# Harrypotterrrr/DVD-GAN

Measured on AMD Instinct MI355X. Metric: clips/sec per G+Ds+Dt step, 48x64x64 UCF-101 synth, higher is better.
Workload: dtype bf16; 1 GPU; UCF-101-shaped 101-class 48x64x64 clips, G+Ds+Dt hinge step, ch=32, k_sample=8, batch 64/GPU (BASELINE configs[1]); global_batch=64, parallelism=dp1

## Files before the change

dvd_gan_amd/csrc/conv_common.h:

```cpp
#pragma once
#include "common.h"

namespace dvdk {

constexpr int BM = 128, BN = 128, NT = 256;
constexpr int TILEB = BM * 80;
constexpr int WG_LD = 132;

__device__ __forceinline__ u32x4 relu16_f32(u32x4 v) {
    v.x = (int32_t)v.x < 0 ? 0u : v.x; v.y = (int32_t)v.y < 0 ? 0u : v.y;
    v.z = (int32_t)v.z < 0 ? 0u : v.z; v.w = (int32_t)v.w < 0 ? 0u : v.w;
    return v;
}
__device__ __forceinline__ uint32_t relu2_bf16(uint32_t v) {
    uint32_t m = ((v >> 15) & 0x00010001u) * 0xffffu;
    return v & ~m;
}
__device__ __forceinline__ u32x4 relu16_bf16(u32x4 v) {
    v.x = relu2_bf16(v.x); v.y = relu2_bf16(v.y); v.z = relu2_bf16(v.z); v.w = relu2_bf16(v.w);
    return v;
}
template <typename T> __device__ __forceinline__ u32x4 relu16(u32x4 v);
template <> __device__ __forceinline__ u32x4 relu16<float>(u32x4 v) { return relu16_f32(v); }
template <> __device__ __forceinline__ u32x4 relu16<bf16_t>(u32x4 v) { return relu16_bf16(v); }
// ... 408 lines not shown
        },
        [&](int i) __attribute__((always_inline)) {
            const int rr = rrow(i);
            float v[8], rv[8], m8[8];
            staged(i, v); unpack8(resv[i % (D + 1)], rv); unpack8(mv[i % (D + 1)], m8);
#pragma unroll
            for (int k = 0; k < 8; ++k) v[k] = (v[k] + bias8[k]) + rv[k];
            if (p.act == DVD_ACT_RELU) {
#pragma unroll
                for (int k = 0; k < 8; ++k) v[k] = fmaxf(v[k], 0.f);
            } else if (p.act == DVD_ACT_TANH) {
#pragma unroll
                for (int k = 0; k < 8; ++k) v[k] = gate_tanh<T>(v[k]);
            } else if (p.act == DVD_ACT_SIGMOID) {
#pragma unroll
                for (int k = 0; k < 8; ++k) v[k] = gate_sigmoid<T>(v[k]);
            }
#pragma unroll
            for (int k = 0; k < 8; ++k) {
                v[k] = (has_mask && !(m8[k] > 0.f)) ? 0.f : v[k];
                v[k] = (k < nvalid) ? v[k] : 0.f;
            }
            if (p.out_f32) bst8<float>(rout, offs(rr, p.ldo, 4, col, colv), v);
            else bst8<T>(rout, offs(rr, p.ldo, esz, col, colv), v);
        });
}

template <bool UP2> struct HaloGeo {
    static constexpr int PITCH = UP2 ? 12 : 20;
    static constexpr int SWA = UP2 ? 2 : 0;
    static __device__ __forceinline__ int sw(int hy, int hx) { return ((hx >> 2) + SWA * hy) & 3; }
};

constexpr int kGroupMax = 6;
struct ConvGroup {
    int n, head, nslots;
    int order[kGroupMax];
    int wgs[kGroupMax];
    ConvK c[kGroupMax];
};
static_assert(sizeof(ConvGroup) <= 3584, "ConvGroup must fit the kernel argument segment");

void launch_gb(const ConvK& p, int variant, bool relu_in, bool up2, dim3 grid, hipStream_t st);
void launch_gbs(const ConvK& p, int S, bool big, bool relu_in, dim3 grid, hipStream_t st);
void launch_group(const ConvGroup& grp, int kind, hipStream_t st);

}
using namespace dvdk;
```

dvd_gan_amd/csrc/conv_gb.hip:

```cpp
#include "conv_common.h"

namespace {

#ifndef DVD_GB_EPI_DEEP
#define DVD_GB_EPI_DEEP 0
#endif

constexpr unsigned kRowOOB = 0x80000000u, kStepOOB = 0x40000000u, kRangeCap = 0x3fffffffu;

template <int TM, int WN, int WMV, bool UP2> struct HaloGbCfg {
    static constexpr int PITCH = HaloGeo<UP2>::PITCH;
    static constexpr int NWAVE = WMV * WN;
    static constexpr int PH = WMV * TM * 2;
    static constexpr int HG = UP2 ? ((PH / 2 + 3) * PITCH + 15) / 16 : ((PH + 4) * PITCH + 15) / 16;
    static constexpr int HBYTES = HG * 1024;
    static constexpr int EPI = NWAVE * 32 * 64 * 4;
    static constexpr int LDSB = 2 * HBYTES + 1024 > EPI ? 2 * HBYTES + 1024 : EPI;
};

template <int TM, bool RELU, class LdA, class Next>
__device__ __forceinline__ void gb_step(f32x16 (&acc)[TM][2], const bf16x8 (&b)[2][2], LdA ldA, Next next) {
    constexpr int NU = 2 * TM;
#ifndef DVD_GB_ADEPTH
#define DVD_GB_ADEPTH 2
// ... 344 lines not shown
                auto next = [&]() __attribute__((always_inline)) {
                    ldBq((ix & 1) ? b0 : b1, nrec);
                    if (ix == 0 && first && more) dmaH(hb ^ 1, cc + 1);
                };
                gb_step<TM, RELU>(acc, (ix & 1) ? b1 : b0, ldA, next);
                rec = nrec;
            }
            ++iy;
            if (last) {
                iy = 0; hb ^= 1; ++cc;
                if (more) {
                    __builtin_amdgcn_s_waitcnt(0xc07f);
                    __builtin_amdgcn_s_barrier();
                }
            }
        };
        const int nrows = nch * KS;
        int r = 0;
#pragma unroll 1
        for (; r + 1 < nrows; r += 2) { row(bq0, bq1); row(bq1, bq0); }
        if (r < nrows) row(bq0, bq1);
    }
    __syncthreads();

    float* ep = reinterpret_cast<float*>(&smem[0]) + wave * (32 * 64);
    const int ecol = (lane & 7) * 8, erow = lane >> 3;
    const long long row0 = (long long)ft0 * SS;
    conv_epilogue<T, TM, DVD_GB_EPI_DEEP>(p, acc, ep, lane, n0 + wn * 64 + ecol, z, ltile, row0, [&](int tm, int j) __attribute__((always_inline)) {
        const int pi = wm * (TM * 32) + tm * 32 + j * 8 + erow;
        return row0 + pi < p.M ? pi : -1;
    });
}

template <int TM, int S, bool RELU, int KS>
__global__ __launch_bounds__(256, 2) void conv_halo_gbs_kernel(ConvK p) {
    __shared__ __attribute__((aligned(16))) char smem[HaloGbsCfg<TM, S>::LDSB];
    const int bid = xcd_order(blockIdx.x, gridDim.x);
    const TileMN t = tile_of(p.nmajor, p.tilesN, bid, gridDim.x);
    conv_halo_gbs_tile<TM, S, RELU, KS>(p, smem, t.mt, t.nt, blockIdx.z, (int)blockIdx.x);
}

template <class TileFn>
__device__ __forceinline__ void group_dispatch(const ConvGroup& grp, TileFn fn) {
    const int x = blockIdx.x & 7;
    int rem = blockIdx.x >> 3;
    auto share = [&](int m) __attribute__((always_inline)) -> int { const int w = grp.wgs[m]; return (w >> 3) + (x < (w & 7) ? 1 : 0); };
    const int m0 = grp.order[0], m1 = grp.n > 1 ? grp.order[1] : m0;
    const int s0 = share(m0), s1 = grp.n > 1 ? share(m1) : 0;
    const int h0 = min(grp.head, s0), h1 = min(grp.head, s1);
    int g = -1, off = 0;
    if (rem < h0) { g = m0; off = rem; }
    else if ((rem -= h0) < h1) { g = m1; off = rem; }
    else if ((rem -= h1) < s0 - h0) { g = m0; off = h0 + rem; }
    else if ((rem -= s0 - h0) < s1 - h1) { g = m1; off = h1 + rem; }
    else {
        rem -= s1 - h1;
        for (int k = 2; k < grp.n; ++k) {
            const int m = grp.order[k], s = share(m);
            if (rem < s) { g = m; off = rem; break; }
            rem -= s;
        }
    }
    if (g < 0) return;
    const int w = grp.wgs[g];
    const int local = x * (w >> 3) + min(x, w & 7) + off;
    const ConvK& p = grp.c[g];
    const int t = local / p.nsplit, z = local - t * p.nsplit;
    const TileMN mn = tile_of(p.nmajor, p.tilesN, t, w / p.nsplit);
    fn(p, mn.mt, mn.nt, z, t);
}

template <int TM, int WN, int WMV>
__global__ __launch_bounds__(256, 2) void conv_group_gb_kernel(ConvGroup grp) {
    __shared__ __attribute__((aligned(16))) char smem[HaloGbCfg<TM, WN, WMV, false>::LDSB];
    group_dispatch(grp, [&](const ConvK& p, int mt, int nt, int z, int t) __attribute__((always_inline)) {
        if (p.kh == 5) conv_halo_gb_tile<TM, WN, WMV, false, false, 5>(p, smem, mt, nt, z, t);
        else conv_halo_gb_tile<TM, WN, WMV, false, false, 3>(p, smem, mt, nt, z, t);
    });
}

template <int TM, int S>
__global__ __launch_bounds__(256, 2) void conv_group_gbs_kernel(ConvGroup grp) {
    __shared__ __attribute__((aligned(16))) char smem[HaloGbsCfg<TM, S>::LDSB];
    group_dispatch(grp, [&](const ConvK& p, int mt, int nt, int z, int t) __attribute__((always_inline)) {
        if (p.kh == 5) conv_halo_gbs_tile<TM, S, false, 5>(p, smem, mt, nt, z, t);
        else conv_halo_gbs_tile<TM, S, false, 3>(p, smem, mt, nt, z, t);
    });
}

struct FragK { const bf16_t* w; bf16_t* wq; int ntaps, Cout, C, kchunks, nb32; };
__global__ void fragment_major_kernel(FragK p) {
    const long long n = (long long)p.ntaps * p.kchunks * p.nb32 * 2 * 64;
    const long long i = (long long)blockIdx.x * blockDim.x + threadIdx.x;
    if (i >= n) return;
    const int l = (int)(i & 63);
    long long r = i >> 6;
    const int kk = (int)(r & 1); r >>= 1;
    const int nb = (int)(r % p.nb32); r /= p.nb32;
    const int cc = (int)(r % p.kchunks);
    const int tap = (int)(r / p.kchunks);
    const int co = nb * 32 + (l & 31), ci = cc * 32 + (kk * 2 + (l >> 5)) * 8;
    u32x4 v = {0u, 0u, 0u, 0u};
    if (co < p.Cout && ci < p.C) v = *reinterpret_cast<const u32x4*>(p.w + ((size_t)tap * p.Cout + co) * p.C + ci);
    *reinterpret_cast<u32x4*>(p.wq + i * 8) = v;
}
constexpr int kFragBatch = 32;
struct FragBatchK { FragK it[kFragBatch]; int first[kFragBatch + 1]; int n; };
__global__ void fragment_major_batched_kernel(FragBatchK b) {
    int j = 0;
    while (j + 1 < b.n && (int)blockIdx.x >= b.first[j + 1]) ++j;
    const FragK& p = b.it[j];
    const long long n = (long long)p.ntaps * p.kchunks * p.nb32 * 2 * 64;
    const long long i = (long long)((int)blockIdx.x - b.first[j]) * blockDim.x + threadIdx.x;
    if (i >= n) return;
    const int l = (int)(i & 63);
    long long r = i >> 6;
    const int kk = (int)(r & 1); r >>= 1;
// ... 1 lines not shown
    const int cc = (int)(r % p.kchunks);
    const int tap = (int)(r / p.kchunks);
    const int co = nb * 32 + (l & 31), ci = cc * 32 + (kk * 2 + (l >> 5)) * 8;
    u32x4 v = {0u, 0u, 0u, 0u};
    if (co < p.Cout && ci < p.C) v = *reinterpret_cast<const u32x4*>(p.w + ((size_t)tap * p.Cout + co) * p.C + ci);
    *reinterpret_cast<u32x4*>(p.wq + i * 8) = v;
}

}

#ifdef DVD_GB_PROBE
namespace dvdk {
void launch_gb(const ConvK& p, int, bool, bool, dim3 grid, hipStream_t st) { conv_halo_gb_kernel<4, 2, 2, false, false, 5><<<grid, 256, 0, st>>>(p); }
void launch_gbs(const ConvK& p, int, bool, bool, dim3 grid, hipStream_t st) { conv_halo_gbs_kernel<2, 8, false, 3><<<grid, 256, 0, st>>>(p); }
void launch_group(const ConvGroup& grp, int, hipStream_t st) { conv_group_gb_kernel<4, 2, 2><<<dim3(grp.nslots), 256, 0, st>>>(grp); }
}
#else
namespace dvdk {
void launch_gb(const ConvK& p, int variant, bool relu_in, bool up2, dim3 grid, hipStream_t st) {
#define LAUNCH_GB4(TM_, WN_, WMV_, KS_)                                                                       \
    do { if (relu_in) { if (up2) conv_halo_gb_kernel<TM_, WN_, WMV_, true, true, KS_><<<grid, 256, 0, st>>>(p);       \
                        else conv_halo_gb_kernel<TM_, WN_, WMV_, true, false, KS_><<<grid, 256, 0, st>>>(p); }           \
         else         { if (up2) conv_halo_gb_kernel<TM_, WN_, WMV_, false, true, KS_><<<grid, 256, 0, st>>>(p);      \
                        else conv_halo_gb_kernel<TM_, WN_, WMV_, false, false, KS_><<<grid, 256, 0, st>>>(p); } } while (0)
#define LAUNCH_GB(TM_, WN_, WMV_) do { if (p.kh == 5) LAUNCH_GB4(TM_, WN_, WMV_, 5); else LAUNCH_GB4(TM_, WN_, WMV_, 3); } while (0)
    if (variant == 2) LAUNCH_GB(2, 1, 4); else if (variant == 0) LAUNCH_GB(4, 2, 2); else LAUNCH_GB(2, 2, 2);
#undef LAUNCH_GB
#undef LAUNCH_GB4
}
void launch_gbs(const ConvK& p, int S, bool big, bool relu_in, dim3 grid, hipStream_t st) {
#define LAUNCH_GBS2(TM_, SZ_, KS_) do { if (relu_in) conv_halo_gbs_kernel<TM_, SZ_, true, KS_><<<grid, 256, 0, st>>>(p);   \
                                        else conv_halo_gbs_kernel<TM_, SZ_, false, KS_><<<grid, 256, 0, st>>>(p); } while (0)
#define LAUNCH_GBS(TM_, SZ_) do { if (p.kh == 5) LAUNCH_GBS2(TM_, SZ_, 5); else LAUNCH_GBS2(TM_, SZ_, 3); } while (0)
    if (S == 8) { if (big) LAUNCH_GBS(4, 8); else LAUNCH_GBS(2, 8); }
    else LAUNCH_GBS(2, 4);
#undef LAUNCH_GBS
#undef LAUNCH_GBS2
}
void launch_group(const ConvGroup& grp, int kind, hipStream_t st) {
    const dim3 grid(grp.nslots);
    switch (kind) {
        case 0: conv_group_gb_kernel<4, 2, 2><<<grid, 256, 0, st>>>(grp); break;
        case 1: conv_group_gb_kernel<2, 2, 2><<<grid, 256, 0, st>>>(grp); break;
        case 2: conv_group_gbs_kernel<4, 8><<<grid, 256, 0, st>>>(grp); break;
        case 3: conv_group_gbs_kernel<2, 8><<<grid, 256, 0, st>>>(grp); break;
        default: conv_group_gbs_kernel<2, 4><<<grid, 256, 0, st>>>(grp); break;
    }
}
}
#endif

extern "C" long long dvd_conv_fragment_major_bytes(int ntaps, int Cout, int C) {
    if (ntaps <= 0 || Cout <= 0 || C <= 0) return 0;
    const long long kchunks = (C + 31) / 32, nb32 = (Cout + 127) / 128 * 4;
    return (long long)ntaps * kchunks * nb32 * 2048;
}
extern "C" int dvd_conv_fragment_major(int dtype, const void* w, void* wq, int ntaps, int Cout, int C, void* stream) {
    if (!w || !wq || ntaps <= 0 || Cout <= 0 || C <= 0) return DVD_E_ARG;
    if (dtype != DVD_BF16 || (C & 7)) return DVD_E_SHAPE;
    FragK p{(const bf16_t*)w, (bf16_t*)wq, ntaps, Cout, C, (C + 31) / 32, (Cout + 127) / 128 * 4};
    const long long n = (long long)ntaps * p.kchunks * p.nb32 * 128;
    fragment_major_kernel<<<cdiv(n, 256), 256, 0, (hipStream_t)stream>>>(p);
    return launch_status();
}

extern "C" int dvd_conv_fragment_major_batched(int dtype, const dvd_frag_item* items, int n, void* stream) {
    if (!items || n <= 0) return DVD_E_ARG;
    if (dtype != DVD_BF16) return DVD_E_SHAPE;
// ... 21 lines not shown
```

dvd_gan_amd/csrc/conv_igemm.hip:

```cpp
#include "conv_common.h"
#include "prof.h"

namespace {

template <typename T, int TM, bool RELU>
__device__ __forceinline__ void mma_swz(const char* At, const char* Bt, int arow, int brow, int lane,
                                        f32x16 (&acc)[TM][2]) {
    const int kh = lane >> 5;
    if constexpr (sizeof(T) == 2) {
#pragma unroll
        for (int kk = 0; kk < 2; ++kk) {
            const int slot = kk * 2 + kh;
            bf16x8 b[2], a[TM];
#pragma unroll
            for (int tn = 0; tn < 2; ++tn) b[tn] = *reinterpret_cast<const bf16x8*>(Bt + lds_off(brow + tn * 32, slot));
#pragma unroll
            for (int tm = 0; tm < TM; ++tm) {
                u32x4 raw = *reinterpret_cast<const u32x4*>(At + lds_off(arow + tm * 32, slot));
                if constexpr (RELU) raw = relu16_bf16(raw);
                a[tm] = __builtin_bit_cast(bf16x8, raw);
            }
#pragma unroll
            for (int tm = 0; tm < TM; ++tm)
#pragma unroll
// ... 470 lines not shown
        stf(reinterpret_cast<T*>(p.wd) + ((size_t)ftap * p.Cip + ci) * p.co_tot_d + p.co_off + co, v);
    }
}

constexpr int kPackBatch = 24;
struct PackBatchK { PackK it[kPackBatch]; int first[kPackBatch + 1]; int n; };
template <typename T>
__global__ void pack_weight_batched_kernel(PackBatchK b) {
    int j = 0;
    while (j + 1 < b.n && (int)blockIdx.x >= b.first[j + 1]) ++j;
    const PackK& p = b.it[j];
    const long long n = (long long)p.Cout * p.Cip * p.ntaps;
    const long long i = (long long)((int)blockIdx.x - b.first[j]) * blockDim.x + threadIdx.x;
    if (i >= n) return;
    const int tap = (int)(i % p.ntaps);
    const long long r = i / p.ntaps;
    const int ci = (int)(r % p.Cip), co = (int)(r / p.Cip);
    float v = 0.f;
    if (ci < p.Cin) {
        v = p.w[((size_t)co * p.ci_tot + p.ci_off + ci) * p.ntaps + tap];
        if (p.sigma) v = v / *p.sigma;
    }
    if (p.wf) stf(reinterpret_cast<T*>(p.wf) + ((size_t)tap * p.co_tot_f + p.co_off + co) * p.Cip + ci, v);
    if (p.wd) {
        const int ftap = p.ntaps - 1 - tap;
        stf(reinterpret_cast<T*>(p.wd) + ((size_t)ftap * p.Cip + ci) * p.co_tot_d + p.co_off + co, v);
    }
}

}

#include <vector>
#include <mutex>
#include <cstdio>
#include <cstdlib>
namespace dvdprof {
bool g_prof = false;
std::vector<ProfRec> g_recs;
std::mutex g_prof_mu;
}
using namespace dvdprof;
extern "C" void dvd_prof_enable(int on) {
    std::lock_guard<std::mutex> l(g_prof_mu);
    g_prof = on != 0;
}
extern "C" long long dvd_prof_report_variants(int kind, int nvar, long long* n, double* ms, double* flops) {
    std::lock_guard<std::mutex> l(g_prof_mu);
    for (int v = 0; v < nvar; ++v) { if (n) n[v] = 0; if (ms) ms[v] = 0; if (flops) flops[v] = 0; }
    long long total = 0;
    std::vector<ProfRec> keep;
    const char* csv = getenv("DVD_PROF_CSV");
    FILE* f = csv ? fopen(csv, "a") : nullptr;
    for (auto& r : g_recs) {
        if (r.kind != kind) { keep.push_back(r); continue; }
        hipEventSynchronize(r.b);
        float t = 0; hipEventElapsedTime(&t, r.a, r.b);
        if (f) fprintf(f, "%d,%lld,%d,%d,%d,%d,%d,%.4f,%.0f,%d\n", r.kind, r.M, r.C, r.Cout, r.taps, r.split, r.flags, t, r.flops, r.variant);
        const int slots[2] = {0, r.variant};
        for (int j = 0; j < (r.variant > 0 ? 2 : 1); ++j) {
            const int v = slots[j];
            if (v >= nvar) continue;
            if (n) ++n[v];
            if (ms) ms[v] += t;
            if (flops) flops[v] += r.flops;
        }
        ++total;
        hipEventDestroy(r.a); hipEventDestroy(r.b);
    }
    if (f) fclose(f);
    g_recs.swap(keep);
    return total;
}
extern "C" long long dvd_prof_report(int kind, double* total_ms, double* total_flops) {
    long long n = 0;
    return dvd_prof_report_variants(kind, 1, &n, total_ms, total_flops);
}

extern "C" int dvd_conv_forward(const dvd_conv_desc* d, void* stream) { return dvd_conv_forward_gru(d, nullptr, stream); }

struct ConvPlan { long long M; bool halo, thin, wide, big, smallf; };
static int conv_plan(const dvd_conv_desc* d, const GruEpi* g, ConvK& p, ConvPlan& pl) {
    if (!d || !d->in || !d->w || (!d->ws && (!d->out || (d->nsplit > 1 && !g)))) return DVD_E_ARG;
    if (g && (d->ws || (g->h & 7) || (d->nsplit > 1 && (!g->slabs || !g->tickets)))) return DVD_E_ARG;
    if (d->frames <= 0 || d->T <= 0 || d->H <= 0 || d->W <= 0 || d->C <= 0 || d->Cout <= 0) return DVD_E_ARG;
    int logH = ilog2_exact(d->H), logW = ilog2_exact(d->W);
    const bool pow2 = logH >= 0 && logW >= 0;
    if (!pow2) logH = logW = -1;
    if ((d->C & 7) || (d->ldi & 7) || !(d->kt & d->kh & d->kw & 1)) return DVD_E_SHAPE;
    if (d->up2 && ((d->H | d->W) & 1)) return DVD_E_SHAPE;
    if (d->kt > 1 && d->up2) return DVD_E_SHAPE;
    const long long M = (long long)d->frames * d->T * d->H * d->W;
    if (M >= (1ll << 31) - BM) return DVD_E_SHAPE;
    p.in = (const char*)d->in; p.w = (const char*)d->w; p.bias = d->bias; p.res = (const char*)d->res;
    p.mask = (const char*)d->mask; p.out = (char*)d->out; p.ws = d->ws; p.wq = (const char*)d->wq;
    p.nb32 = (d->Cout + 127) / 128 * 4;
    p.M = (int)M; p.C = d->C; p.ldi = d->ldi; p.Cout = d->Cout; p.ldo = d->ldo; p.ldres = d->ldres; p.ldmask = d->ldmask;
    p.res_up2 = d->res && d->res_up2;
    if (p.res_up2 && (d->H < 2 || d->W < 2 || ((d->H | d->W) & 1))) return DVD_E_SHAPE;
    p.T = d->T; p.H = d->H; p.W = d->W; p.logH = logH; p.logW = logW;
    p.Hin = d->up2 ? d->H / 2 : d->H; p.Win = d->up2 ? d->W / 2 : d->W;
    p.kt = d->kt; p.kh = d->kh; p.kw = d->kw;
    const int bk = d->dtype == DVD_BF16 ? 32 : 16;
    p.kchunks = (d->C + bk - 1) / bk;
    p.nk = d->kt * d->kh * d->kw * p.kchunks;
    p.nsplit = d->nsplit < 1 ? 1 : d->nsplit;
    if (p.nsplit > p.nk) p.nsplit = p.nk;
    if (p.nsplit != (d->nsplit < 1 ? 1 : d->nsplit)) return DVD_E_ARG;
    const long long t256 = cdiv(M, 256) * (long long)cdiv(d->Cout, 256) * p.nsplit;
    const int rem256 = d->Cout % 256;
    const bool halo = pow2 && d->kh == d->kw && (d->kh == 3 || d->kh == 5) && d->W >= 16 && d->H >= 16 &&
                      p.nsplit <= p.kchunks * d->kt;
// ... 2 lines not shown
                        p.nsplit <= p.kchunks && M < (1ll << 24);
    const bool thin = halo && d->dtype == DVD_BF16 && d->Cout <= 64 && cdiv(M, 256) * (long long)p.nsplit >= 512;
    const bool wide = !halo && !smallf && d->dtype == DVD_BF16 && d->Cout >= 256 && (rem256 == 0 || rem256 > 224) && t256 >= 256 &&
                      !(g && p.nsplit > 1);
    p.tilesN = wide ? (d->Cout + 255) / 256 : thin ? 1 : (d->Cout + BN - 1) / BN;
    p.up2 = d->up2; p.relu_in = d->relu_in; p.act = d->act; p.out_f32 = d->out_f32;
    if (g) p.g = *g; else p.g = GruEpi{};
    p.nmajor = 0;
    {
        const size_t esz = d->dtype == DVD_BF16 ? 2 : 4;
        const size_t rows_in = (size_t)d->frames * d->T * p.Hin * p.Win;
        const size_t inb = ((rows_in - 1) * (size_t)d->ldi + d->C) * esz;
        const size_t wb = (size_t)d->kt * d->kh * d->kw * d->Cout * d->C * esz;
        if (wb >= 0xffffffffull) return DVD_E_SHAPE;
        p.in_bytes = inb; p.w_bytes = (unsigned)wb;
        p.maxshift = ((d->kt >> 1) * d->H + (d->kh >> 1)) * d->W + (d->kw >> 1);
        p.nmajor = !halo && wb > inb && wb > (4u << 20);
        if (halo && p.tilesN > 1 && wb > ((size_t)5 << 20)) p.nmajor = 1;
        if (halo && p.tilesN >= 6 && wb > (2u << 20)) p.nmajor = 1;
    }
    constexpr long long big_thr = 512;
    const bool one_tap = d->kt * d->kh * d->kw == 1 && !halo && !smallf;
    const bool big = wide || (cdiv(M, 256) * (long long)p.tilesN * p.nsplit >= big_thr && !one_tap);
    p.pm = 0;
    {
        const int bmt = (wide || big) ? 256 : 128;
        const int F = d->frames;
        const bool lines = (F % bmt == 0) || (bmt % F == 0 && d->W % (bmt / F) == 0);
        const size_t esz = d->dtype == DVD_BF16 ? 2 : 4;
        if (!halo && !smallf && pow2 && d->kt == 1 && d->T == 1 && !d->up2 && d->kh >= 3 && d->H <= 8 && lines &&
            (size_t)M * (size_t)(d->ldi > 3 * d->Cout ? d->ldi : 3 * d->Cout) * 4 < (1ull << 31))
            p.pm = F;
    }
    pl.M = M; pl.halo = halo; pl.thin = thin; pl.wide = wide; pl.big = big && !(smallf && d->W == 4); pl.smallf = smallf;
    p.pool2 = d->pool2 != 0;
    if (p.pool2 && (!halo || p.nsplit != 1 || g || d->ws || d->res || d->act != DVD_ACT_NONE || d->kt != 1 || d->T != 1 || d->up2))
        return DVD_E_SHAPE;
    return DVD_OK;
}

extern "C" int dvd_conv_pool2_ok(const dvd_conv_desc* d) {
    if (!d || !d->pool2) return 0;
    ConvK p; ConvPlan pl;
    dvd_conv_desc t = *d;
    static char dummy;
    if (!t.out) t.out = &dummy;
    return conv_plan(&t, nullptr, p, pl) == DVD_OK ? 1 : 0;
}

extern "C" int dvd_conv_forward_gru(const dvd_conv_desc* d, const GruEpi* g, void* stream) {
    ConvK p; ConvPlan pl;
    const int rc = conv_plan(d, g, p, pl);
    if (rc != DVD_OK) return rc;
    const long long M = pl.M;
    const bool halo = pl.halo, thin = pl.thin, wide = pl.wide, big = pl.big;
    if (d->wq_kind >= 2 && !(d->wq_kind == 2 ? dvd_conv_thin_in_ok(d) : dvd_conv_thin_out_ok(d))) return DVD_E_ARG;
    if (d->wq_kind >= 2 && d->pool2) return DVD_E_ARG;
    if (!g && d->wq && d->wq_kind == 2 && dvd_conv_thin_in_ok(d)) {
        ProfScope prof(0, 2.0 * (double)M * d->Cout * d->C * d->kt * d->kh * d->kw, stream, M, d->C, d->Cout, d->kt * d->kh * d->kw, 1,
                       d->relu_in << 1);
        prof.r.variant = 9;
        return dvd_conv_thin_in(d, stream);
    }
    if (!g && d->wq && d->wq_kind == 3 && dvd_conv_thin_out_ok(d)) {
        ProfScope prof(0, 2.0 * (double)M * d->Cout * d->C * d->kt * d->kh * d->kw, stream, M, d->C, d->Cout, d->kt * d->kh * d->kw, 1,
                       d->relu_in << 1);
// ... 55 lines not shown
    if (!d || !g || n < 1 || n > kGroupMax || kind < 0 || kind > 4) return DVD_E_ARG;
    ConvGroup grp = {};
    grp.n = n;
    double flops = 0; long long Msum = 0;
    for (int i = 0; i < n; ++i) {
        ConvPlan pl;
        const GruEpi* gi = g[i].mode ? &g[i] : nullptr;
        const int rc = conv_plan(&d[i], gi, grp.c[i], pl);
        if (rc != DVD_OK) return rc;
        ConvK& p = grp.c[i];
        if (d[i].dtype != DVD_BF16 || !p.wq || d[i].wq_kind > 1 || d[i].relu_in || d[i].up2 || d[i].ws) return DVD_E_ARG;
        long long mtiles;
        if (kind <= 1) {
            if (!pl.halo || d[i].H < (kind == 0 ? 16 : 8)) return DVD_E_SHAPE;
            mtiles = cdiv(pl.M, kind == 0 ? 256 : 128);
        } else {
            const int S = kind == 4 ? 4 : 8;
            if (!pl.smallf || d[i].W != S) return DVD_E_SHAPE;
            mtiles = cdiv(d[i].frames, kind == 2 ? 4 : kind == 3 ? 2 : 8);
        }
        p.tilesN = (d[i].Cout + BN - 1) / BN;
        const long long tiles = mtiles * p.tilesN;
        if (p.nsplit > 1) {
            if (!gi || tiles > 1024) return DVD_E_SHAPE;
            p.g.tickets += i * 1024;
        }
        if (tiles * p.nsplit > (1 << 20)) return DVD_E_SHAPE;
        grp.wgs[i] = (int)(tiles * p.nsplit);
        flops += 2.0 * (double)pl.M * d[i].Cout * d[i].C * d[i].kh * d[i].kw;
        Msum += pl.M;
    }
    {
        long long len[kGroupMax];
        for (int i = 0; i < n; ++i) { grp.order[i] = i; len[i] = (long long)grp.c[i].kchunks * d[i].kh * d[i].kw / grp.c[i].nsplit; }
        for (int i = 1; i < n; ++i)
            for (int j = i; j > 0 && len[grp.order[j]] > len[grp.order[j - 1]]; --j) { const int t = grp.order[j]; grp.order[j] = grp.order[j - 1]; grp.order[j - 1] = t; }
        long long slots = 0;
        for (int i = 0; i < n; ++i) slots += (grp.wgs[i] + 7) / 8;
        grp.nslots = (int)(8 * slots);
        grp.head = run > 0 ? run : run < 0 ? 0 : 32;
    }
    ProfScope prof(0, flops, stream, Msum, d[0].C, d[0].Cout, d[0].kh * d[0].kw, n, 0);
    prof.r.variant = kind <= 1 ? 10 : 11;
    launch_group(grp, kind, (hipStream_t)stream);
    return launch_status();
}

extern "C" int dvd_conv_wants_fragment_major(const dvd_conv_desc* d) {
    ConvK p; ConvPlan pl;
    dvd_conv_desc t = *d;
    if (!t.w) t.w = t.in;
    t.wq = t.w;
    if (conv_plan(&t, nullptr, p, pl) != DVD_OK) return 0;
    if (dvd_conv_thin_in_ok(d)) return 2;
    if (dvd_conv_thin_out_ok(d)) return 3;
    return ((pl.halo || pl.smallf) && d->dtype == DVD_BF16) ? 1 : 0;
}

extern "C" int dvd_pack_conv_weight(int dtype, const float* w, const float* sigma, int Cout, int Cin, int ntaps,
                                    int Cip, int co_off, int co_tot_f, int co_tot_d, void* wf, void* wd,
                                    int kt, int kh, int kw, int ci_off, int ci_tot, void* stream) {
    if (!w || (!wf && !wd) || Cout <= 0 || Cin <= 0 || ntaps != kt * kh * kw) return DVD_E_ARG;
    if (ci_tot <= 0) { ci_off = 0; ci_tot = Cin; }
    if (ci_off < 0 || ci_off + Cin > ci_tot) return DVD_E_ARG;
    if ((Cip & 7) || Cip < Cin || (wd && (co_tot_d & 7))) return DVD_E_SHAPE;
    PackK p{w, sigma, (char*)wf, (char*)wd, Cout, Cin, ntaps, Cip, co_off, co_tot_f, co_tot_d, kt, kh, kw, ci_off, ci_tot};
    const long long n = (long long)Cout * Cip * ntaps;
// ... 36 lines not shown
```

dvd_gan_amd/csrc/gru.hip:

```cpp
#include "common.h"
#include <algorithm>
#include <atomic>
#include <cstdlib>
#include <cstring>
#include <map>
#include <mutex>
#include <queue>
#include <string>
#include <vector>

namespace {


__device__ __forceinline__ void slab_sum8(const float* ws, int ns, size_t stride, size_t off, float (&acc)[8]) {
    int s = 0;
    for (; s + 4 <= ns; s += 4) {
        float a[4][8];
#pragma unroll
        for (int j = 0; j < 4; ++j) load8<float>(ws + (size_t)(s + j) * stride + off, a[j]);
#pragma unroll
        for (int j = 0; j < 4; ++j)
#pragma unroll
            for (int k = 0; k < 8; ++k) acc[k] += a[j][k];
    }
// ... 381 lines not shown
    if (!s || s->n_layers < 1 || s->n_layers > DVD_GRU_STACK_MAX) return DVD_E_ARG;
    const dvd_gru_desc& a = s->layer[0];
    if (a.dtype != DVD_BF16 || a.T <= 0 || a.B <= 0 || !a.tickets || !s->ws) return DVD_E_ARG;
    if (stack_kind(s) < 0) return DVD_E_SHAPE;
    for (int l = 0; l < s->n_layers; ++l) {
        const dvd_gru_desc& d = s->layer[l];
        if (d.dtype != a.dtype || d.T != a.T || d.B != a.B || d.H != a.H || d.W != a.W) return DVD_E_ARG;
        if (d.hidden <= 0 || (d.hidden & 7) || (d.k != 3 && d.k != 5)) return DVD_E_SHAPE;
        if ((long long)d.B * d.H * d.W * (d.hidden / 8) >= (1ll << 31)) return DVD_E_SHAPE;
        if (!d.gx || !d.h_all || !d.u_all || !d.hr_all) return DVD_E_ARG;
        if (l > 0 && (s->cin[l] != s->layer[l - 1].hidden || d.gx_stride != (long long)d.B * d.H * d.W * 3 * d.hidden)) return DVD_E_ARG;
        if (!backward) {
            if (!d.w_ur || !d.w_o || !d.w_ur_q || !d.w_o_q) return DVD_E_ARG;
            if (!d.infer && (!d.r_all || !d.o_all)) return DVD_E_ARG;
            if (l > 0 && (!s->wx[l] || !s->wx_q[l] || !s->bx[l])) return DVD_E_ARG;
        } else {
            if (!d.wd_ur || !d.wd_o || !d.wd_ur_q || !d.wd_o_q || !d.r_all || !d.o_all || !d.dg || !d.carry) return DVD_E_ARG;
            if (l > 0 && (!s->wdx[l] || !s->wdx_q[l] || !s->dh_mid[l])) return DVD_E_ARG;
        }
    }
    return DVD_OK;
}

void member_conv(Member& m, const dvd_gru_desc& L, const void* in, int C, int ldi, const void* w, const void* wq, int Cout, int kind) {
    m = Member{};
    dvd_conv_desc& d = m.d;
    d.dtype = L.dtype; d.frames = L.B; d.T = 1; d.H = L.H; d.W = L.W; d.C = C; d.ldi = ldi; d.Cout = Cout; d.ldo = Cout;
    d.kt = 1; d.kh = L.k; d.kw = L.k; d.nsplit = 1; d.in = in; d.w = w; d.wq = wq; d.wq_kind = 1;
    m.tiles = kind_mtiles(kind, L.B, L.H, L.W) * cdiv(Cout, 128);
    m.kchunks = (C + 31) / 32;
}

struct SplitPlan { int ns[2 * DVD_GRU_STACK_MAX]; };
double model_makespan(int n, const long long* tiles, const int* units, const int* ns, int slots, double fixed, double split_cost) {
    int order[2 * DVD_GRU_STACK_MAX];
    double len[2 * DVD_GRU_STACK_MAX];
    for (int i = 0; i < n; ++i) { order[i] = i; len[i] = (double)units[i] / ns[i] + fixed + (ns[i] > 1 ? split_cost : 0.0); }
    std::sort(order, order + n, [&](int a, int b) { return (double)units[a] / ns[a] > (double)units[b] / ns[b]; });
    std::priority_queue<double, std::vector<double>, std::greater<double>> q;
    for (int i = 0; i < slots; ++i) q.push(0.0);
    double end = 0.0;
    for (int oi = 0; oi < n; ++oi) {
        const int i = order[oi];
        const long long w = (tiles[i] * ns[i] + 7) / 8;
        for (long long k = 0; k < w; ++k) {
            const double t = q.top() + len[i];
            q.pop(); q.push(t);
            if (t > end) end = t;
        }
    }
    return end;
}
SplitPlan plan_splits(int kind, bool backward, int n, const Member* m, long long cap) {
    static std::map<std::string, SplitPlan> cache;
    static std::mutex mu;
    long long tiles[2 * DVD_GRU_STACK_MAX]; int units[2 * DVD_GRU_STACK_MAX], capi[2 * DVD_GRU_STACK_MAX];
    std::string key;
    key.append((const char*)&kind, sizeof kind); key.push_back(backward ? 1 : 0);
    for (int i = 0; i < n; ++i) {
        tiles[i] = m[i].tiles; units[i] = m[i].kchunks * m[i].d.kh * m[i].d.kw;
        capi[i] = (int)std::min<long long>(cap, m[i].kchunks);
        if (m[i].tiles > 1024) capi[i] = 1;
        key.append((const char*)&tiles[i], sizeof tiles[i]); key.append((const char*)&units[i], sizeof units[i]);
        key.append((const char*)&capi[i], sizeof capi[i]);
    }
    std::lock_guard<std::mutex> lock(mu);
    auto it = cache.find(key);
    if (it != cache.end()) return it->second;
    const int slots = (kind == 0 || kind == 2) ? 64 : 96;
    double fixed = (kind == 0 || kind == 2) ? 12.0 : 16.0;
    double split_cost = kind == 4 ? 3.0 : kind == 0 ? 150.0 : backward ? 50.0 : 80.0;
#ifdef DVD_STACK_SEARCH_DEBUG
    if (const char* e = getenv("DVD_SS_FIXED")) fixed = atof(e);
    if (const char* e = getenv("DVD_SS_SPLIT")) split_cost = atof(e);
#endif
    static const int opts[] = {1, 2, 3, 4, 8};
    SplitPlan best{}; double best_t = 1e30;
    int idx[2 * DVD_GRU_STACK_MAX] = {0};
    if (n > 5) {
        int ns[2 * DVD_GRU_STACK_MAX];
        for (int i = 0; i < n; ++i) ns[i] = 1;
        auto cost = [&]() { int k = 0; for (int i = 0; i < n; ++i) k += ns[i] > 1;
                            return model_makespan(n, tiles, units, ns, slots, fixed, split_cost) * (1.0 + 0.004 * k); };
        best_t = cost();
        for (bool moved = true; moved;) {
            moved = false;
            for (int i = 0; i < n; ++i) {
                const int keep = ns[i]; int pick = keep;
                for (int o : opts) {
                    if (o > capi[i] || o == keep) continue;
                    ns[i] = o;
                    const double t = cost();
                    if (t < best_t * (1.0 - 1e-9)) { best_t = t; pick = o; moved = true; }
                }
                ns[i] = pick;
            }
        }
        for (int i = 0; i < n; ++i) best.ns[i] = ns[i];
    } else
    for (;;) {
        int ns[2 * DVD_GRU_STACK_MAX]; bool ok = true; int nsplit_members = 0;
        for (int i = 0; i < n; ++i) { ns[i] = opts[idx[i]]; if (ns[i] > capi[i]) ok = false; nsplit_members += ns[i] > 1; }
        if (ok) {
            const double t = model_makespan(n, tiles, units, ns, slots, fixed, split_cost) * (1.0 + 0.004 * nsplit_members);
            if (t < best_t) { best_t = t; for (int i = 0; i < n; ++i) best.ns[i] = ns[i]; }
        }
        int j = 0;
        while (j < n && ++idx[j] == (int)(sizeof opts / sizeof opts[0])) idx[j++] = 0;
        if (j == n) break;
    }
#ifdef DVD_STACK_SEARCH_DEBUG
    {
        int one[2 * DVD_GRU_STACK_MAX]; for (int i = 0; i < n; ++i) one[i] = 1;
        fprintf(stderr, "plan kind %d %s:", kind, backward ? "bwd" : "fwd");
        for (int i = 0; i < n; ++i) fprintf(stderr, " [tiles %lld units %d cap %d -> ns %d]", tiles[i], units[i], capi[i], best.ns[i]);
        fprintf(stderr, "  model %.0f (unsplit %.0f)\n", best_t, model_makespan(n, tiles, units, one, slots, fixed, split_cost));
    }
#endif
    cache[key] = best;
    return best;
}

int run_group(const dvd_gru_stack_desc* s, int kind, Member* m, GruEpi* g, int n, void* stream, bool dry, long long& ws_need, bool backward) {
    if (n == 0) return DVD_OK;
    long long total = 0;
    for (int i = 0; i < n; ++i) total += m[i].tiles;
    const long long cap = (kind == 4 && backward) ? 8 : 4;
    const long long target = (kind == 0 || kind == 2) ? 512 : 768;
    long long want = (target + total - 1) / total;
    if (want > cap) want = cap;
    SplitPlan plan{};
    bool searched = !s->layer_policy && DVD_STACK_SEARCH_KINDS(kind);
#ifdef DVD_STACK_SEARCH_DEBUG
    if (const char* e = getenv("DVD_SS_MASK")) searched = searched && ((atoi(e) >> kind) & 1) && ((atoi(e) >> (backward ? 9 : 8)) & 1);
#endif
    if (searched) plan = plan_splits(kind, backward, n, m, cap);
    long long cursor = 0;
    dvd_conv_desc d[kMaxMember];
    for (int i = 0; i < n; ++i) {
        long long ns = searched ? plan.ns[i] : want;
        if (s->layer_policy)
            ns = m[i].gate ? dvd_conv_pick_nsplit(DVD_BF16, (long long)m[i].d.frames * m[i].d.H * m[i].d.W, m[i].d.Cout, m[i].d.C,
                                                  m[i].d.kh * m[i].d.kw) : 1;
        if (s->layer[0].ns_cap > 0 && ns > s->layer[0].ns_cap) ns = s->layer[0].ns_cap;
        if (ns > m[i].kchunks) ns = m[i].kchunks;
        if (ns > 1 && m[i].tiles > 1024) ns = 1;
        m[i].d.nsplit = (int)ns;
        if (ns > 1) {
            if (g[i].mode == 0) g[i].mode = 6;
            g[i].slabs = s->ws + cursor; g[i].tickets = s->layer[0].tickets;
            cursor += ns * m[i].tiles * kind_tile_floats(kind);
        }
        d[i] = m[i].d;
    }
    if (dry) {
        if (cursor > ws_need) ws_need = cursor;
        return DVD_OK;
    }
    for (long long seen = g_ws_high.load(); cursor > seen && !g_ws_high.compare_exchange_weak(seen, cursor);) {}
    if (cursor > ws_need) return DVD_E_SHAPE;
// ... 215 lines not shown
```

include/dvdgan_hip.h:

```cpp
#ifndef DVDGAN_HIP_H
#define DVDGAN_HIP_H
#include <stdint.h>
#ifdef __cplusplus
extern "C" {
#endif
#pragma GCC visibility push(default)

#define DVD_F32 0
#define DVD_BF16 1

#define DVD_OK 0
#define DVD_E_ARG (-1)
#define DVD_E_SHAPE (-2)
#define DVD_E_LAUNCH (-3)

#define DVD_ACT_NONE 0
#define DVD_ACT_RELU 1
#define DVD_ACT_TANH 2
#define DVD_ACT_SIGMOID 3

int dvd_abi_version(void);
#define DVD_STRUCT_CONV 0
#define DVD_STRUCT_WGRAD 1
#define DVD_STRUCT_GRU 2
// ... 8 lines not shown
const char* dvd_strerror(int code);

typedef struct {
    int dtype;
    int frames, T, H, W;
    int C, ldi;
    int Cout, ldo;
    int kt, kh, kw;
    int up2;
    int relu_in;
    int nsplit;
    int act;
    int out_f32;
    int ldres, ldmask;
    int res_up2;
    const void* in;
    const void* w;
    const float* bias;
    const void* res;
    const void* mask;
    void* out;
    float* ws;
    const void* wq;
    int wq_kind;
    int pool2;
} dvd_conv_desc;
int dvd_conv_forward(const dvd_conv_desc* d, void* stream);
int dvd_conv_pool2_ok(const dvd_conv_desc* d);
long long dvd_conv_fragment_major_bytes(int ntaps, int Cout, int C);
int dvd_conv_fragment_major(int dtype, const void* w, void* wq, int ntaps, int Cout, int C, void* stream);
typedef struct { const void* w; void* wq; int ntaps, Cout, C; } dvd_frag_item;
int dvd_conv_fragment_major_batched(int dtype, const dvd_frag_item* items, int n, void* stream);
int dvd_conv_wants_fragment_major(const dvd_conv_desc* d);
long long dvd_conv_thin_image_bytes(int kt);
int dvd_conv_thin_image(const void* w, void* wt, int kt, void* stream);
long long dvd_conv_thin_out_image_bytes(void);
int dvd_conv_thin_out_image(const void* w, void* wt, int rows, void* stream);

typedef struct {
    int dtype;
    int frames, T, H, W;
    int C, ldx;
    int Cin_real;
    int Cout, Cy, ldy;
    int kt, kh, kw;
    int up2, relu_in;
    int msplit;
    long long s_co, s_ci, s_tap;
    const void* x;
    const void* dy;
    float* dw;
    float* dbias;
    float* ws;
    int overwrite;
} dvd_wgrad_desc;
int dvd_conv_wgrad(const dvd_wgrad_desc* d, void* stream);
long long dvd_conv_wgrad_ws_floats(const dvd_wgrad_desc* d);

int dvd_pack_conv_weight(int dtype, const float* w, const float* sigma, int Cout, int Cin, int ntaps,
                         int Cip, int co_off, int co_tot_f, int co_tot_d, void* wf, void* wd,
                         int kt, int kh, int kw, int ci_off, int ci_tot, void* stream);
typedef struct {
    const float* w; const float* sigma; void* wf; void* wd;
    int Cout, Cin, ntaps, Cip, co_off, co_tot_f, co_tot_d, kt, kh, kw, ci_off, ci_tot;
} dvd_pack_item;
int dvd_pack_conv_weight_batched(int dtype, const dvd_pack_item* items, int n, void* stream);
// ... 171 lines not shown
```

Before: 144.3 clips/s.

## Add pixel-major line4 kernel for 4x4 convs skipping out-of-frame taps

Adds a new conv tile path for 4x4 spatial frames (the GRU kind-4 convs). It organizes each tile as one image row across 32 frames, so only the kernel rows and columns that overlap the frame are computed and loaded, instead of all KS*KS taps. The split planner and group ordering are updated to model per-line step counts, and the split caps for these layers are lowered. This adds kernel complexity and a larger LDS footprint in the grouped kernel, and it can be turned off through an env var.

```diff
diff --git a/dvd_gan_amd/csrc/conv_common.h b/dvd_gan_amd/csrc/conv_common.h
--- a/dvd_gan_amd/csrc/conv_common.h
+++ b/dvd_gan_amd/csrc/conv_common.h
@@ -464,6 +464,14 @@
     static __device__ __forceinline__ int sw(int hy, int hx) { return ((hx >> 2) + SWA * hy) & 3; }
 };
 
+struct Line4 {
+    static constexpr __host__ __device__ int row_lo(int KS, int y) { return (KS >> 1) > y ? (KS >> 1) - y : 0; }
+    static constexpr __host__ __device__ int row_hi(int KS, int y) { return 3 + (KS >> 1) - y < KS - 1 ? 3 + (KS >> 1) - y : KS - 1; }
+    static constexpr __host__ __device__ int rows(int KS, int y) { return row_hi(KS, y) - row_lo(KS, y) + 1; }
+    static constexpr __host__ __device__ int cols(int KS) { return KS == 5 ? 4 : KS; }
+    static constexpr __host__ __device__ int steps(int KS, int y) { return rows(KS, y) * cols(KS); }
+};
+
 constexpr int kGroupMax = 6;
 struct ConvGroup {
     int n, head, nslots;
diff --git a/dvd_gan_amd/csrc/conv_gb.hip b/dvd_gan_amd/csrc/conv_gb.hip
--- a/dvd_gan_amd/csrc/conv_gb.hip
+++ b/dvd_gan_amd/csrc/conv_gb.hip
@@ -400,12 +400,167 @@
     });
 }
 
-template <int TM, int S, bool RELU, int KS>
+struct Line4Cfg {
+    static constexpr int ROWB = 32 * 64;
+    static constexpr int HBYTES = 16 * ROWB;
+    static constexpr int LDSB = ROWB + 2 * HBYTES + 1024;
+};
+
+template <bool RELU, int KS>
+__device__ __forceinline__ void conv_line4_gbs_tile(const ConvK& p, char* const smem, const int mt, const int nt, const int z, const int ltile) {
+    using T = bf16_t;
+    constexpr int TM = 2, WN = 2, BNt = 128, SS = 16;
+    constexpr int ROWB = Line4Cfg::ROWB, HBYTES = Line4Cfg::HBYTES;
+    constexpr int ntap2 = KS * KS, pad = KS >> 1, NTX = Line4::cols(KS);
+    char* const zeros = &smem[0];
+    char* const hbuf0 = &smem[ROWB];
+    char* const dump = &smem[ROWB + 2 * HBYTES];
+    const int tid = threadIdx.x, lane = tid & 63, wave = tid >> 6;
+    const int wn = wave % WN;
+    const int n0 = nt * BNt;
+    const int y = mt & 3, ft0 = (mt >> 2) * 32;
+    const int per = (p.kchunks + p.nsplit - 1) / p.nsplit;
+    const int cc_begin = z * per, cc_end = min(p.kchunks, cc_begin + per);
+    constexpr unsigned esz = 2;
+
+    const int wu = __builtin_amdgcn_readfirstlane(wave);
+    const int wm = wu >> 1;
+    const int iy_lo = Line4::row_lo(KS, y), iy_hi = Line4::row_hi(KS, y), nl = iy_hi - iy_lo + 1;
+    const int ylo = y + iy_lo - pad;
+    const int ix0 = KS == 5 ? 1 - wm : 0;
+    const int xb = 2 * wm + ix0 - pad;
+
+    const unsigned ldb = (unsigned)p.ldi * esz;
+    const size_t base_b = (size_t)ft0 * SS * ldb;
+    const size_t left_b = p.in_bytes - base_b;
+    const __amdgpu_buffer_rsrc_t rin = __builtin_amdgcn_make_buffer_rsrc(
+        (void*)(p.in + base_b), 0, left_b > kRangeCap ? kRangeCap : (unsigned)left_b, 0x00020000);
+    const int nb32 = p.nb32;
+    const __amdgpu_buffer_rsrc_t rwq = __builtin_amdgcn_make_buffer_rsrc(
+        (void*)p.wq, 0, (unsigned)((size_t)ntap2 * p.kchunks * nb32 * 2048), 0x00020000);
+    const int hq = (lane & 3) ^ (lane >> 4);
+    const unsigned dbase = (unsigned)((((wu & 1) * 16 + (lane >> 2)) * SS + ylo * 4 + (wu >> 1)) * ldb) + hq * 16;
+    const bool ragged = (p.C & 31) != 0;
+    auto dmaH = [&](int hb, int cc_) __attribute__((always_inline)) {
+        unsigned lo_ = dbase + cc_ * 64;
+        if (ragged && cc_ == p.kchunks - 1) lo_ = cc_ * 32 + hq * 8 < p.C ? lo_ : kRowOOB;
+#pragma unroll
+        for (int i = 0; i < 8; ++i) {
+            const int line = i >> 1;
+            const bool on = line < nl;
+            char* dst_ = on ? hbuf0 + hb * HBYTES + (i * 4 + wu) * 1024 : dump;
+            const unsigned off_ = on ? lo_ + (unsigned)(line * 4 + (i & 1) * 2) * ldb : kRowOOB;
+            dma16(rin, dst_, off_);
+        }
+    };
+    const unsigned bvoff = (unsigned)(wn * 2 * 2048 + lane * 16);
+    const unsigned bnt = (unsigned)(nt * (BNt / 32)) * 2048u;
+    const unsigned brec = (unsigned)nb32 * 2048u;
+    const unsigned tapstep = (unsigned)p.kchunks * brec;
+    auto ldBq = [&](bf16x8 (&b)[2][2], unsigned rec) __attribute__((always_inline)) {
+#pragma unroll
+        for (int kk = 0; kk < 2; ++kk)
+#pragma unroll
+            for (int tn = 0; tn < 2; ++tn)
+                b[kk][tn] = __builtin_bit_cast(bf16x8, __builtin_amdgcn_raw_buffer_load_b128(rwq, bvoff, rec + (unsigned)(tn * 2048 + kk * 1024), 0));
+    };
+    auto rec0 = [&](int cc_) __attribute__((always_inline)) -> unsigned {
+        return ((unsigned)(iy_lo * KS + ix0) * p.kchunks + cc_) * brec + bnt;
+    };
+
+    f32x16 acc[TM][2];
+    {
+        const f32x16 zacc = {0.f, 0.f, 0.f, 0.f, 0.f, 0.f, 0.f, 0.f, 0.f, 0.f, 0.f, 0.f, 0.f, 0.f, 0.f, 0.f};
+#pragma unroll
+        for (int a = 0; a < TM; ++a)
+#pragma unroll
+            for (int b = 0; b < 2; ++b) acc[a][b] = zacc;
+    }
+    const int l31 = lane & 31, kh2 = lane >> 5;
+    const int swz = (l31 >> 2) & 3;
+    const int alane[2] = {l31 * 64 + ((kh2 ^ swz) << 4), l31 * 64 + (((2 + kh2) ^ swz) << 4)};
+#ifdef DVD_EXP_NOMAIN
+    const int nch = 0;
+#else
+    const int nch = cc_end - cc_begin;
+#endif
+    if (nch > 0) {
+        unsigned rec = rec0(cc_begin);
+        bf16x8 bq0[2][2], bq1[2][2];
+        *reinterpret_cast<uint2*>(zeros + tid * 8) = uint2{0u, 0u};
+        dmaH(0, cc_begin);
+        ldBq(bq0, rec);
+        __builtin_amdgcn_s_waitcnt(0x0070);
+        __builtin_amdgcn_s_barrier();
+        int hb = 0, iy = iy_lo, cc = cc_begin;
+        auto row = [&](bf16x8 (&b0)[2][2], bf16x8 (&b1)[2][2]) __attribute__((always_inline)) {
+            const bool first = iy == iy_lo, last = iy == iy_hi, more = cc + 1 < cc_end;
+            const char* const Arow = hbuf0 + hb * HBYTES + ((iy - iy_lo) * 4 + xb) * ROWB;
+#pragma unroll
+            for (int j = 0; j < NTX; ++j) {
+                auto ldA = [&](int u) __attribute__((always_inline)) -> bf16x8 {
+                    const int kk = u / TM, tm = u % TM;
+                    const char* base = Arow + (j + tm) * ROWB;
+                    if (j == 0 && tm == 0) base = wm == 0 ? zeros : base;
+                    if (j == NTX - 1 && tm == 1) base = wm == 1 ? zeros : base;
+                    return *reinterpret_cast<const bf16x8*>(base + alane[kk]);
+                };
+                unsigned nrec = rec + tapstep;
+                if (j == NTX - 1) {
+                    nrec = rec + (unsigned)(1 + KS - NTX) * tapstep;
+                    if (last) nrec = more ? rec0(cc + 1) : rec;
+                }
+                auto next = [&]() __attribute__((always_inline)) {
+                    ldBq((j & 1) ? b0 : b1, nrec);
+                    if (j == 0 && first && more) dmaH(hb ^ 1, cc + 1);
+                };
+                gb_step<TM, RELU>(acc, (j & 1) ? b1 : b0, ldA, next);
+                rec = nrec;
+            }
+            ++iy;
+            if (last) {
+                iy = iy_lo; hb ^= 1; ++cc;
+                if (more) {
+                    __builtin_amdgcn_s_waitcnt(0xc07f);
+                    __builtin_amdgcn_s_barrier();
+                }
+            }
+        };
+        const int nrows = nch * nl;
+        int r = 0;
+        if constexpr (NTX & 1) {
+#pragma unroll 1
+            for (; r + 1 < nrows; r += 2) { row(bq0, bq1); row(bq1, bq0); }
+            if (r < nrows) row(bq0, bq1);
+        } else {
+#pragma unroll 1
+            for (; r < nrows; ++r) row(bq0, bq1);
+        }
+    }
+    __syncthreads();
+
+    float* ep = reinterpret_cast<float*>(&smem[0]) + wave * (32 * 64);
+    const int ecol = (lane & 7) * 8, erow = lane >> 3;
+    const long long row0 = (long long)ft0 * SS;
+    const int prow = y * 4 + wm * 2;
+    conv_epilogue<T, TM, DVD_GB_EPI_DEEP>(p, acc, ep, lane, n0 + wn * 64 + ecol, z, ltile, row0, [&](int tm, int j) __attribute__((always_inline)) {
+        const int rr = (j * 8 + erow) * SS + prow + tm;
+        return row0 + rr < p.M ? rr : -1;
+    });
+}
+
+template <int TM, int S> struct GbsLds {
+    static constexpr int A = HaloGbsCfg<TM, S>::LDSB, B = (S == 4) ? Line4Cfg::LDSB : 0;
+    static constexpr int LDSB = A > B ? A : B;
+};
+
+template <int TM, int S, bool RELU, int KS, bool PM = false>
 __global__ __launch_bounds__(256, 2) void conv_halo_gbs_kernel(ConvK p) {
-    __shared__ __attribute__((aligned(16))) char smem[HaloGbsCfg<TM, S>::LDSB];
+    __shared__ __attribute__((aligned(16))) char smem[PM ? Line4Cfg::LDSB : HaloGbsCfg<TM, S>::LDSB];
     const int bid = xcd_order(blockIdx.x, gridDim.x);
     const TileMN t = tile_of(p.nmajor, p.tilesN, bid, gridDim.x);
-    conv_halo_gbs_tile<TM, S, RELU, KS>(p, smem, t.mt, t.nt, blockIdx.z, (int)blockIdx.x);
+    if constexpr (PM) conv_line4_gbs_tile<RELU, KS>(p, smem, t.mt, t.nt, blockIdx.z, (int)blockIdx.x);
+    else conv_halo_gbs_tile<TM, S, RELU, KS>(p, smem, t.mt, t.nt, blockIdx.z, (int)blockIdx.x);
 }
 
 template <class TileFn>
@@ -449,8 +604,15 @@
 
 template <int TM, int S>
 __global__ __launch_bounds__(256, 2) void conv_group_gbs_kernel(ConvGroup grp) {
-    __shared__ __attribute__((aligned(16))) char smem[HaloGbsCfg<TM, S>::LDSB];
+    __shared__ __attribute__((aligned(16))) char smem[GbsLds<TM, S>::LDSB];
     group_dispatch(grp, [&](const ConvK& p, int mt, int nt, int z, int t) __attribute__((always_inline)) {
+        if constexpr (S == 4) {
+            if (p.pm > 0) {
+                if (p.kh == 5) conv_line4_gbs_tile<false, 5>(p, smem, mt, nt, z, t);
+                else conv_line4_gbs_tile<false, 3>(p, smem, mt, nt, z, t);
+                return;
+            }
+        }
         if (p.kh == 5) conv_halo_gbs_tile<TM, S, false, 5>(p, smem, mt, nt, z, t);
         else conv_halo_gbs_tile<TM, S, false, 3>(p, smem, mt, nt, z, t);
     });
@@ -518,8 +680,12 @@
 #define LAUNCH_GBS2(TM_, SZ_, KS_) do { if (relu_in) conv_halo_gbs_kernel<TM_, SZ_, true, KS_><<<grid, 256, 0, st>>>(p);   \
                                         else conv_halo_gbs_kernel<TM_, SZ_, false, KS_><<<grid, 256, 0, st>>>(p); } while (0)
 #define LAUNCH_GBS(TM_, SZ_) do { if (p.kh == 5) LAUNCH_GBS2(TM_, SZ_, 5); else LAUNCH_GBS2(TM_, SZ_, 3); } while (0)
+#define LAUNCH_LINE4(KS_) do { if (relu_in) conv_halo_gbs_kernel<2, 4, true, KS_, true><<<grid, 256, 0, st>>>(p);   \
+                               else conv_halo_gbs_kernel<2, 4, false, KS_, true><<<grid, 256, 0, st>>>(p); } while (0)
     if (S == 8) { if (big) LAUNCH_GBS(4, 8); else LAUNCH_GBS(2, 8); }
+    else if (p.pm > 0) { if (p.kh == 5) LAUNCH_LINE4(5); else LAUNCH_LINE4(3); }
     else LAUNCH_GBS(2, 4);
+#undef LAUNCH_LINE4
 #undef LAUNCH_GBS
 #undef LAUNCH_GBS2
 }
diff --git a/dvd_gan_amd/csrc/conv_igemm.hip b/dvd_gan_amd/csrc/conv_igemm.hip
--- a/dvd_gan_amd/csrc/conv_igemm.hip
+++ b/dvd_gan_amd/csrc/conv_igemm.hip
@@ -526,6 +526,8 @@
 
 #include <vector>
 #include <mutex>
+#include <atomic>
+#include <cstring>
 #include <cstdio>
 #include <cstdlib>
 namespace dvdprof {
@@ -571,6 +573,25 @@
 }
 
 extern "C" int dvd_conv_forward(const dvd_conv_desc* d, void* stream) { return dvd_conv_forward_gru(d, nullptr, stream); }
+
+static std::atomic<int> g_frame_rows{-1};
+static bool small_frame_rows_by_frame() {
+    int v = g_frame_rows.load(std::memory_order_relaxed);
+    if (v < 0) {
+        const char* e = getenv("DVD_SMALL_FRAME_ROWS");
+        v = (e && !strcmp(e, "frame")) ? 1 : 0;
+        g_frame_rows.store(v, std::memory_order_relaxed);
+    }
+    return v != 0;
+}
+extern "C" void dvd_debug_small_frame_rows(int by_frame) { g_frame_rows.store(by_frame ? 1 : 0, std::memory_order_relaxed); }
+extern "C" int dvd_conv_small_tile_pixel_major(int S, int frames) {
+    return S == 4 && frames > 0 && frames % 32 == 0 && !small_frame_rows_by_frame();
+}
+extern "C" int dvd_conv_small_tile_steps(int S, int KS, int line) {
+    if ((S != 4 && S != 8) || (KS != 3 && KS != 5) || line < 0 || line >= S) return 0;
+    return S == 4 ? Line4::steps(KS, line) : KS * KS;
+}
 
 struct ConvPlan { long long M; bool halo, thin, wide, big, smallf; };
 static int conv_plan(const dvd_conv_desc* d, const GruEpi* g, ConvK& p, ConvPlan& pl) {
@@ -639,6 +660,7 @@
             (size_t)M * (size_t)(d->ldi > 3 * d->Cout ? d->ldi : 3 * d->Cout) * 4 < (1ull << 31))
             p.pm = F;
     }
+    if (smallf && dvd_conv_small_tile_pixel_major(d->W, d->frames)) p.pm = d->frames;
     pl.M = M; pl.halo = halo; pl.thin = thin; pl.wide = wide; pl.big = big && !(smallf && d->W == 4); pl.smallf = smallf;
     p.pool2 = d->pool2 != 0;
     if (p.pool2 && (!halo || p.nsplit != 1 || g || d->ws || d->res || d->act != DVD_ACT_NONE || d->kt != 1 || d->T != 1 || d->up2))
@@ -760,7 +782,10 @@
     }
     {
         long long len[kGroupMax];
-        for (int i = 0; i < n; ++i) { grp.order[i] = i; len[i] = (long long)grp.c[i].kchunks * d[i].kh * d[i].kw / grp.c[i].nsplit; }
+        for (int i = 0; i < n; ++i) {
+            const int steps = grp.c[i].pm > 0 ? Line4::steps(d[i].kh, 1) : d[i].kh * d[i].kw;
+            grp.order[i] = i; len[i] = (long long)grp.c[i].kchunks * steps / grp.c[i].nsplit;
+        }
         for (int i = 1; i < n; ++i)
             for (int j = i; j > 0 && len[grp.order[j]] > len[grp.order[j - 1]]; --j) { const int t = grp.order[j]; grp.order[j] = grp.order[j - 1]; grp.order[j - 1] = t; }
         long long slots = 0;
diff --git a/dvd_gan_amd/csrc/gru.hip b/dvd_gan_amd/csrc/gru.hip
--- a/dvd_gan_amd/csrc/gru.hip
+++ b/dvd_gan_amd/csrc/gru.hip
@@ -437,7 +437,8 @@
 }
 
 struct SplitPlan { int ns[2 * DVD_GRU_STACK_MAX]; };
-double model_makespan(int n, const long long* tiles, const int* units, const int* ns, int slots, double fixed, double split_cost) {
+double model_makespan(int n, const long long* tiles, const int* units, const int* ns, int slots, double fixed, double split_cost,
+                      const int (*lines)[4] = nullptr, const int* tilesN = nullptr) {
     int order[2 * DVD_GRU_STACK_MAX];
     double len[2 * DVD_GRU_STACK_MAX];
     for (int i = 0; i < n; ++i) { order[i] = i; len[i] = (double)units[i] / ns[i] + fixed + (ns[i] > 1 ? split_cost : 0.0); }
@@ -449,7 +450,8 @@
         const int i = order[oi];
         const long long w = (tiles[i] * ns[i] + 7) / 8;
         for (long long k = 0; k < w; ++k) {
-            const double t = q.top() + len[i];
+            const double cut = lines ? (double)(units[i] - lines[i][(k / ns[i] / tilesN[i]) & 3]) / ns[i] : 0.0;
+            const double t = q.top() + len[i] - cut;
             q.pop(); q.push(t);
             if (t > end) end = t;
         }
@@ -462,8 +464,16 @@
     long long tiles[2 * DVD_GRU_STACK_MAX]; int units[2 * DVD_GRU_STACK_MAX], capi[2 * DVD_GRU_STACK_MAX];
     std::string key;
     key.append((const char*)&kind, sizeof kind); key.push_back(backward ? 1 : 0);
+    int lines[2 * DVD_GRU_STACK_MAX][4], tilesN[2 * DVD_GRU_STACK_MAX];
+    const bool pixmajor = kind == 4 && dvd_conv_small_tile_pixel_major(4, m[0].d.frames);
+    key.push_back(pixmajor ? 1 : 0);
     for (int i = 0; i < n; ++i) {
-        tiles[i] = m[i].tiles; units[i] = m[i].kchunks * m[i].d.kh * m[i].d.kw;
+        tiles[i] = m[i].tiles; units[i] = 0;
+        for (int y = 0; y < 4; ++y) {
+            lines[i][y] = m[i].kchunks * (pixmajor ? dvd_conv_small_tile_steps(4, m[i].d.kh, y) : m[i].d.kh * m[i].d.kw);
+            units[i] = std::max(units[i], lines[i][y]);
+        }
+        tilesN[i] = (int)cdiv(m[i].d.Cout, 128);
         capi[i] = (int)std::min<long long>(cap, m[i].kchunks);
         if (m[i].tiles > 1024) capi[i] = 1;
         key.append((const char*)&tiles[i], sizeof tiles[i]); key.append((const char*)&units[i], sizeof units[i]);
@@ -486,7 +496,7 @@
         int ns[2 * DVD_GRU_STACK_MAX];
         for (int i = 0; i < n; ++i) ns[i] = 1;
         auto cost = [&]() { int k = 0; for (int i = 0; i < n; ++i) k += ns[i] > 1;
-                            return model_makespan(n, tiles, units, ns, slots, fixed, split_cost) * (1.0 + 0.004 * k); };
+                            return model_makespan(n, tiles, units, ns, slots, fixed, split_cost, pixmajor ? lines : nullptr, tilesN) * (1.0 + 0.004 * k); };
         best_t = cost();
         for (bool moved = true; moved;) {
             moved = false;
@@ -507,7 +517,7 @@
         int ns[2 * DVD_GRU_STACK_MAX]; bool ok = true; int nsplit_members = 0;
         for (int i = 0; i < n; ++i) { ns[i] = opts[idx[i]]; if (ns[i] > capi[i]) ok = false; nsplit_members += ns[i] > 1; }
         if (ok) {
-            const double t = model_makespan(n, tiles, units, ns, slots, fixed, split_cost) * (1.0 + 0.004 * nsplit_members);
+            const double t = model_makespan(n, tiles, units, ns, slots, fixed, split_cost, pixmajor ? lines : nullptr, tilesN) * (1.0 + 0.004 * nsplit_members);
             if (t < best_t) { best_t = t; for (int i = 0; i < n; ++i) best.ns[i] = ns[i]; }
         }
         int j = 0;
@@ -530,7 +540,14 @@
     if (n == 0) return DVD_OK;
     long long total = 0;
     for (int i = 0; i < n; ++i) total += m[i].tiles;
-    const long long cap = (kind == 4 && backward) ? 8 : 4;
+#ifndef DVD_GRU4_CAP_FWD
+#define DVD_GRU4_CAP_FWD 3
+#endif
+#ifndef DVD_GRU4_CAP_BWD
+#define DVD_GRU4_CAP_BWD 4
+#endif
+    const bool line4 = kind == 4 && dvd_conv_small_tile_pixel_major(4, m[0].d.frames);
+    const long long cap = line4 ? (backward ? DVD_GRU4_CAP_BWD : DVD_GRU4_CAP_FWD) : (kind == 4 && backward) ? 8 : 4;
     const long long target = (kind == 0 || kind == 2) ? 512 : 768;
     long long want = (target + total - 1) / total;
     if (want > cap) want = cap;
diff --git a/include/dvdgan_hip.h b/include/dvdgan_hip.h
--- a/include/dvdgan_hip.h
+++ b/include/dvdgan_hip.h
@@ -64,6 +64,9 @@
 typedef struct { const void* w; void* wq; int ntaps, Cout, C; } dvd_frag_item;
 int dvd_conv_fragment_major_batched(int dtype, const dvd_frag_item* items, int n, void* stream);
 int dvd_conv_wants_fragment_major(const dvd_conv_desc* d);
+int dvd_conv_small_tile_steps(int S, int KS, int line);
+int dvd_conv_small_tile_pixel_major(int S, int frames);
+void dvd_debug_small_frame_rows(int by_frame);
 long long dvd_conv_thin_image_bytes(int kt);
 int dvd_conv_thin_image(const void* w, void* wt, int kt, void* stream);
 long long dvd_conv_thin_out_image_bytes(void);
```

Result: no change. 144.7 clips/s (median of 6 runs) (+0.3%).
